# Whitby-Li/monoORBSLAM3

Measured on AMD Instinct MI355X. Metric: ORB extract+match frames/s @1242×375, 2000 feat; 1/2/4/8 GPU + %HBM roofline, higher is better.
Workload: dtype u8; 1 GPU; KITTI 1242x375, 2000 feat, 8-level pyramid scale 1.2, FAST 20/7; extract + 2000x2000 Hamming best-2 per frame; width=1242, height=375, n_features=2000, match=True, records=False, match_placement=after-fast, parallelism=512 resident frame(s) on one GPU, no collective

## Files before the change

### include/orbx.h

```cpp
#ifndef ORBX_H
#define ORBX_H

#include <stddef.h>
#include <stdint.h>

#ifdef __cplusplus
extern "C" {
#endif

#define ORBX_OK 0
#define ORBX_E_ARG (-1)
#define ORBX_E_NO_DEVICE (-2)
#define ORBX_E_CAPACITY (-3)
#define ORBX_E_UNSUPPORTED (-4)

#define ORBX_MAX_LEVELS 16

typedef struct orbx_kp {
    float x, y;
    float size;
    float angle;
    float response;
    int32_t octave;
    int32_t class_id;
// ... 38 lines not shown
int orbx_stream_wait_fast(orbx_t *h, void *stream);
int orbx_synchronize(orbx_t *h);
int orbx_host_register(void *ptr, size_t bytes);
int orbx_host_unregister(void *ptr);

int orbx_tap_level(orbx_t *h, int frame, int level, int blurred, uint8_t *out, size_t out_bytes);
int orbx_tap_candidates(orbx_t *h, int frame, int level, uint16_t *xs, uint16_t *ys, uint8_t *resp,
                        int cap, int *n_out);
int orbx_tap_level_counts(orbx_t *h, int frame, int32_t *counts);

int orbx_tap_sincos(orbx_t *h, const float *angles_deg, int n, float *cos_sin);

#define ORBX_VAR_FAST 0
#define ORBX_VAR_BLUR 1
#define ORBX_VAR_RESIZE_LDS 2
#define ORBX_VAR_RESIZE2 3
#define ORBX_VAR_SIDE_BLUR 4
#define ORBX_VAR_EARLY_FAST 5
#define ORBX_VAR_SPLIT_LEVEL0 6
#define ORBX_VAR_STREAMS 7
#define ORBX_VAR_ZERO_COPY 8
#define ORBX_VAR_DESC 9
#define ORBX_VAR_FAST_CELL_GROUP 10
#define ORBX_N_VARIANTS 11
int orbx_set_variant(orbx_t *h, int which, int value);
int orbx_get_variant(const orbx_t *h, int which, int *value);

#define ORBX_STAGE_RESIZE 0
#define ORBX_STAGE_FAST 1
#define ORBX_STAGE_BLUR 2
#define ORBX_STAGE_OCTREE 3
#define ORBX_STAGE_ORIENT 4
#define ORBX_STAGE_DESC 5
#define ORBX_N_STAGES 6
int orbx_set_stage_timing(orbx_t *h, int enable);
int orbx_stage_times_in_step_ms(orbx_t *h, float *ms );
int orbx_fast_times_in_step_ms(orbx_t *h, float *ms_sum, int *n_launches);
int orbx_stage_times_ms(orbx_t *h, float *ms );

const char *orbx_last_error(void);
const char *orbx_version(void);

#ifdef __cplusplus
}
#endif
#endif
```

### monoorbslam3_amd/csrc/orbx_api.hip

```cpp
#include <math.h>
#include <stdio.h>
#include <stdlib.h>
#include <string.h>

#include <algorithm>
#include <map>
#include <mutex>
#include <string>
#include <vector>

#include "orb_host.h"
#include "orb_math.h"
#include "orbx_internal.h"

static thread_local std::string g_err;
int orbx_set_error(int code, const std::string &msg) { g_err = msg; return code; }

hipError_t orbx_lds_opt_in(const void *kernel, size_t bytes)
{
    static std::mutex mu;
    static std::map<std::pair<const void *, int>, size_t> configured;
    int dev = 0;
    hipError_t e = hipGetDevice(&dev);
    if (e != hipSuccess) return e;
// ... 10 lines not shown
        sel, kp_ang, sel_count, sel_prefix, l0_stage;
};

struct orbx_ctx {
    orbx_cfg cfg;
    HandleStream hs;
    int n_cus = ORBX_N_CUS;
    float scale_factors[ORBX_MAX_LEVELS], inv_scale_factors[ORBX_MAX_LEVELS];
    float square_sigmas[ORBX_MAX_LEVELS], inv_square_sigmas[ORBX_MAX_LEVELS];
    float log_scale_factor;
    int quotas[ORBX_MAX_LEVELS];
    int u_max[ORBX_HALF_PATCH + 1];
    int taps[7];
    int cur_w, cur_h;
    OrbxLevels levels;
    size_t l0_stage_pitch;
    OrbxArenas arena;
    OrbxBuffers buf;
    DevBuf d_levels;
    DevBuf d_xtap[ORBX_MAX_LEVELS], d_ytap[ORBX_MAX_LEVELS];
    bool resize2_ok[ORBX_MAX_LEVELS];
    bool resize_lds_ok[ORBX_MAX_LEVELS];
    int resize_lds;
    int resize2;
    DevBuf d_umax, d_taps;
    hipEvent_t ev_after_fast; bool after_fast_valid;
    hipEvent_t ev_in[ORBX_N_STAGES][4]; int ev_in_n[ORBX_N_STAGES];
    DevBuf d_fast_cells; int n_fast_cells;
    DevBuf d_fast_strips; int n_fast_strips, n_fast_strips0;
    int fast_variant;
    int zero_copy;
    int fast_cell_group;
    int desc_variant;
    DevBuf d_blur_tiles; int n_blur_tiles;
    DevBuf d_blur_strips, d_band_h, d_band_v;
    BlurMfmaLevels blur_tab; int blur_strips_before[ORBX_MAX_LEVELS + 1]; int blur_mfma_levels;
    DevBuf d_bd_blocks, d_bd_band_h; int n_bd_blocks, bd_levels, bd_bk_stride;
    BdLevels bd_tab;
    DevBuf d_bd_bk_start, d_bd_items;
    int alloc_bd_batch, alloc_bd_kcap, alloc_bd_stride;
    int last_fused_levels;
    int blur_mfma;
    size_t l0_stage_fs;
    DevBuf d_slot_level;
    DevBuf d_out_block; PinBuf h_out_block; uint8_t *h_out_dev; size_t out_block_bytes, out_kp_off, out_desc_off;
    orbx_kp *d_out_kp; uint8_t *d_out_desc; int32_t *d_out_n;
// ... 67 lines not shown
}

static void linear_taps(int dn, int sn, bool clamp_ofs, std::vector<OrbxTap> &out)
{
    out.resize(dn);
    const double inv_scale = (double)dn / sn;
    const double scale = 1. / inv_scale;
    for (int d = 0; d < dn; ++d) {
        float f = (float)((d + 0.5) * scale - 0.5);
        int s = orb_floor_f(f);
        f -= (float)s;
        if (clamp_ofs) {
            if (s < 0) { f = 0; s = 0; }
            if (s >= sn - 1) { f = 0; s = sn - 1; }
        }
        auto sat = [](int v) { return (int16_t)std::min(std::max(v, -32768), 32767); };
        out[d].ofs = s;
        out[d].c0 = sat(orb_round_f((1.f - f) * 2048.f));
        out[d].c1 = sat(orb_round_f(f * 2048.f));
    }
}

static size_t align_up(size_t v, size_t a) { return (v + a - 1) / a * a; }
#ifndef ORBX_SIDE_FIRST_PIXELS
#define ORBX_SIDE_FIRST_PIXELS 1200000ull
#endif
#ifndef ORBX_FUSED_DESC_MIN_PIXELS
#define ORBX_FUSED_DESC_MIN_PIXELS 55000000ull
#endif

struct Geometry {
    OrbxLevels levels;
    size_t img_fs, cand_fs, node_fs, l0_fs;
    int l0_pitch;
    size_t sort_lds;
};

static int compute_geometry(const orbx_ctx *c, int w0, int h0, Geometry *g)
{
    memset(g, 0, sizeof *g);
    OrbxLevels &LV = g->levels;
    LV.n_levels = c->cfg.n_levels;
    LV.ini_th = c->cfg.ini_th_fast;
    LV.min_th = c->cfg.min_th_fast;
    size_t img = 0, cand = 0, node = 0;
    int kp = 0, max_quota = 1;
// ... 166 lines not shown
            std::vector<uint8_t> bh, bv;
            orbx_build_blur_mfma(c->levels, c->taps, bs, bh, bv, c->blur_tab, c->blur_strips_before);
            c->blur_mfma_levels = orbx_blur_mfma_levels(c->levels);
            ORB_TRY(upload(c->d_blur_strips, bs, 2));
            ORB_TRY(upload(c->d_band_h, bh, 16));
            ORB_TRY(upload(c->d_band_v, bv, 16));
            std::vector<uint16_t> bb;
            std::vector<uint8_t> bdh;
            orbx_build_blur_desc(c->levels, c->taps, c->blur_tab, bb, bdh, c->bd_tab, &c->bd_levels, &c->bd_bk_stride);
            c->n_bd_blocks = (int)(bb.size() / 2);
            ORB_TRY(upload(c->d_bd_blocks, bb, 2));
            ORB_TRY(upload(c->d_bd_band_h, bdh, 16));
        }
        std::vector<OrbxTap> taps, ytaps;
        for (int l = 1; l < c->levels.n_levels; ++l) {
            const OrbxLevel &d = c->levels.lv[l], &s = c->levels.lv[l - 1];
            linear_taps(d.w, s.w, true, taps);
            while (taps.size() % 4) taps.push_back(taps.back());
            ORB_TRY(upload(c->d_xtap[l], taps));
            linear_taps(d.h, s.h, false, ytaps);
            ORB_TRY(upload(c->d_ytap[l], ytaps));
            c->resize2_ok[l - 1] = l >= 2 && orbx_resize2_fits(taps.data(), ytaps.data(), s.w, s.h, d.w, d.h);
            c->resize_lds_ok[l] = orbx_resize_lds_fits(taps.data(), ytaps.data(), s.w, s.h, d.w, d.h);
        }
    }
    if (c->alloc_batch > c->alloc_bd_batch || c->levels.kcap_total > c->alloc_bd_kcap || c->bd_bk_stride > c->alloc_bd_stride) {
        ORB_TRY(hipDeviceSynchronize());
        c->alloc_bd_batch = std::max(c->alloc_batch, c->alloc_bd_batch);
        c->alloc_bd_kcap = std::max(c->levels.kcap_total, c->alloc_bd_kcap);
        c->alloc_bd_stride = std::max(c->bd_bk_stride, c->alloc_bd_stride);
        ORB_TRY(need_exact<int>(c->d_bd_bk_start, (size_t)c->alloc_bd_stride * c->alloc_bd_batch));
        ORB_TRY(need_exact<uint8_t>(c->d_bd_items, (size_t)32 * std::max(c->alloc_bd_kcap, 1) * c->alloc_bd_batch));
    }
    c->buf.img_frame_stride = c->alloc_img_fs;
    c->buf.cand_frame_stride = c->alloc_cand_fs;
    c->buf.node_frame_stride = c->alloc_node_fs;
    c->l0_stage_fs = c->alloc_l0_fs;
    return ORBX_OK;
}

static int create_common(const orbx_cfg *cfg, const int *quotas_override, orbx_t **out)
{
    if (!cfg || !out) return orbx_set_error(ORBX_E_ARG, "null argument");
    *out = nullptr;
    if (cfg->n_levels < 1 || cfg->n_levels > ORBX_MAX_LEVELS) return orbx_set_error(ORBX_E_ARG, "n_levels out of range");
    if (cfg->n_features < 1) return orbx_set_error(ORBX_E_ARG, "n_features must be >= 1");
// ... 18 lines not shown
        return cleanup(orbx_set_error(ORBX_E_NO_DEVICE, "hipStreamCreate failed"));
    for (int i = 0; i <= ORBX_N_STAGES; ++i)
        if (hipEventCreate(&c->ev[i]) != hipSuccess) return cleanup(orbx_set_error(ORBX_E_NO_DEVICE, "hipEventCreate failed"));
    for (int i = 0; i < 8; ++i)
        if (hipStreamCreateWithFlags(&c->sub[i], hipStreamNonBlocking) != hipSuccess ||
            hipEventCreateWithFlags(&c->ev_join[i], hipEventDisableTiming) != hipSuccess)
            return cleanup(orbx_set_error(ORBX_E_NO_DEVICE, "sub-stream creation failed"));
    if (hipEventCreateWithFlags(&c->ev_fork, hipEventDisableTiming) != hipSuccess)
        return cleanup(orbx_set_error(ORBX_E_NO_DEVICE, "hipEventCreate failed"));
    for (int i = 0; i < 9; ++i)
        if (hipStreamCreateWithFlags(&c->side[i], hipStreamNonBlocking) != hipSuccess ||
            hipEventCreateWithFlags(&c->ev_pyr[i], hipEventDisableTiming) != hipSuccess ||
            hipEventCreateWithFlags(&c->ev_blur[i], hipEventDisableTiming) != hipSuccess ||
            hipEventCreateWithFlags(&c->ev_start[i], hipEventDisableTiming) != hipSuccess ||
            hipEventCreateWithFlags(&c->ev_fast0[i], hipEventDisableTiming) != hipSuccess)
            return cleanup(orbx_set_error(ORBX_E_NO_DEVICE, "side-stream creation failed"));
    c->side_blur = 1;
    c->early_fast = -1;
    c->split_level0 = 1;
    c->fast_variant = 0;
    c->blur_mfma = 1;
    c->resize2 = 1;
    c->resize_lds = 1;
    c->n_sub = 1;
    c->zero_copy = 1;
    c->desc_variant = 0;
    c->fast_cell_group = 8;
    if (need_exact<OrbxLevels>(c->d_levels, 1) != hipSuccess || need_exact<int>(c->d_umax, 16) != hipSuccess ||
        need_exact<int>(c->d_taps, 8) != hipSuccess)
        return cleanup(orbx_set_error(ORBX_E_NO_DEVICE, "hipMalloc failed"));
    if (hipMemcpy(c->d_umax.p, c->u_max, sizeof(int) * 16, hipMemcpyHostToDevice) != hipSuccess ||
        hipMemcpy(c->d_taps.p, c->taps, sizeof(int) * 7, hipMemcpyHostToDevice) != hipSuccess)
        return cleanup(orbx_set_error(ORBX_E_NO_DEVICE, "hipMemcpy failed"));
    if (cfg->max_width > 0 && cfg->max_height > 0) {
        int rc = ensure_geometry(c, cfg->max_width, cfg->max_height, c->cfg.max_batch, 0);
        if (rc) return cleanup(rc);
    }
    *out = c;
    return ORBX_OK;
}

extern "C" int orbx_create(const orbx_cfg *cfg, orbx_t **out) { return create_common(cfg, nullptr, out); }


extern "C" int orbx_create_requota(const orbx_t *other, int n_features, orbx_t **out)
{
// ... 98 lines not shown
    const OrbxBuffers b = offset_buffers(c->buf, f0, LV.kcap_total);
    const OrbxLevels *d_levels = c->d_levels.as<OrbxLevels>();
    auto xtap = [&](int l) { return c->d_xtap[l].as<OrbxTap>(); };
    auto ytap = [&](int l) { return c->d_ytap[l].as<OrbxTap>(); };
    d_l0 += (size_t)f0 * l0_fs;
    d_kp += (size_t)f0 * cap; d_desc += (size_t)f0 * cap * 32; d_n += f0;
    if (t) ORB_TRY(hipEventRecord(c->ev[0], s));
    auto raw = [&](int l, const uint8_t **p, size_t *fs, int *pitch) {
        if (l == 0) { *p = d_l0; *fs = l0_fs; *pitch = l0_pitch; }
        else { *p = b.img_arena + LV.lv[l].raw_off; *fs = b.img_frame_stride; *pitch = LV.lv[l].pitch; }
    };
    const bool lds_resize = c->resize_lds == 2 || (c->resize_lds == 1 && (size_t)n_frames * (size_t)LV.lv[0].w * (size_t)LV.lv[0].h >= (size_t)100000000);
    auto launch_resize = [&](hipStream_t st, int l, int *zero_counts) -> int {
        const uint8_t *sp; size_t sfs; int spitch;
        raw(l - 1, &sp, &sfs, &spitch);
        if ((c->resize2 == 2 || (c->resize2 == 1 && n_frames < 24)) && l + 1 < L && c->resize2_ok[l] && LV.lv[l - 1].w >= 8) {
            orbx_launch_resize2(st, sp, sfs, spitch, LV.lv[l - 1].w, LV.lv[l - 1].h, b.img_arena + LV.lv[l].raw_off, b.img_frame_stride,
                                LV.lv[l].pitch, LV.lv[l].w, LV.lv[l].h, xtap(l), ytap(l), b.img_arena + LV.lv[l + 1].raw_off,
                                b.img_frame_stride, LV.lv[l + 1].pitch, LV.lv[l + 1].w, LV.lv[l + 1].h, xtap(l + 1),
                                ytap(l + 1), n_frames, zero_counts);
            return l + 1;
        }
        if (lds_resize && c->resize_lds_ok[l]) {
            orbx_launch_resize_lds(st, sp, sfs, spitch, LV.lv[l - 1].w, LV.lv[l - 1].h, l == 1 ? LV.lv[0].w : spitch,
                                   b.img_arena + LV.lv[l].raw_off, b.img_frame_stride, LV.lv[l].pitch, LV.lv[l].w, LV.lv[l].h, xtap(l),
                                   ytap(l), n_frames, zero_counts);
            return l;
        }
        orbx_launch_resize(st, sp, sfs, spitch, LV.lv[l - 1].w, LV.lv[l - 1].h, b.img_arena + LV.lv[l].raw_off, b.img_frame_stride,
                           LV.lv[l].pitch, LV.lv[l].w, LV.lv[l].h, xtap(l), ytap(l), n_frames, zero_counts);
        return l;
    };
    const bool side_ok = !t && c->side_blur && slot >= 0;
    const bool strips = c->fast_variant == 2 || (c->fast_variant == 0 && n_frames >= 24);
    const uint16_t *d_units = (strips ? c->d_fast_strips : c->d_fast_cells).as<uint16_t>();
    const int n_units = strips ? c->n_fast_strips : c->n_fast_cells;
    const int n_cells0 = strips ? c->n_fast_strips0 : LV.lv[0].n_cols * LV.lv[0].n_rows;
    auto launch_fast = [&](hipStream_t st, const uint16_t *units, int n) {
        InStep ft(c, ORBX_STAGE_FAST, st);
        if (strips) orbx_launch_fast_strips(st, d_l0, l0_fs, l0_pitch, d_levels, LV, b, units, n, n_frames);
        else orbx_launch_fast(st, d_l0, l0_fs, l0_pitch, d_levels, LV, b, units, n, n_frames, c->fast_cell_group);
    };
    const bool big_call = (size_t)n_frames * (size_t)LV.lv[0].w * (size_t)LV.lv[0].h >= (size_t)ORBX_FUSED_DESC_MIN_PIXELS;
    const int fl = (c->desc_variant == 2 || (c->desc_variant == 0 && big_call)) ? c->bd_levels : 0;
    c->last_fused_levels = fl;
    auto launch_blur = [&](hipStream_t st, int lb, int le) {
        lb = std::max(lb, fl);
        if (le <= lb) return;
        InStep bt(c, ORBX_STAGE_BLUR, st);
// ... 398 lines not shown
{
    if (!c || !ms) return orbx_set_error(ORBX_E_ARG, "null argument");
    if (!c->ev_valid) return orbx_set_error(ORBX_E_ARG, "no timed extract call yet");
    ORB_TRY(hipSetDevice(c->hs.device));
    ORB_TRY(hipEventSynchronize(c->ev[ORBX_N_STAGES]));
    for (int i = 0; i < ORBX_N_STAGES; ++i) ORB_TRY(hipEventElapsedTime(&ms[i], c->ev[i], c->ev[i + 1]));
    return ORBX_OK;
}

static int *variant_field(orbx_ctx *c, int which, int *lo, int *hi)
{
    switch (which) {
    case ORBX_VAR_FAST: *lo = 0; *hi = 2; return &c->fast_variant;
    case ORBX_VAR_BLUR: *lo = 0; *hi = 2; return &c->blur_mfma;
    case ORBX_VAR_RESIZE_LDS: *lo = 0; *hi = 2; return &c->resize_lds;
    case ORBX_VAR_RESIZE2: *lo = 0; *hi = 2; return &c->resize2;
    case ORBX_VAR_SIDE_BLUR: *lo = 0; *hi = 3; return &c->side_blur;
    case ORBX_VAR_EARLY_FAST: *lo = -1; *hi = 2; return &c->early_fast;
    case ORBX_VAR_SPLIT_LEVEL0: *lo = 0; *hi = ORBX_MAX_LEVELS; return &c->split_level0;
    case ORBX_VAR_STREAMS: *lo = 1; *hi = 8; return &c->n_sub;
    case ORBX_VAR_ZERO_COPY: *lo = 0; *hi = 1; return &c->zero_copy;
    case ORBX_VAR_DESC: *lo = 0; *hi = 2; return &c->desc_variant;
    case ORBX_VAR_FAST_CELL_GROUP: *lo = 1; *hi = 16; return &c->fast_cell_group;
    default: return nullptr;
    }
}

extern "C" int orbx_set_variant(orbx_t *c, int which, int value)
{
    if (!c) return orbx_set_error(ORBX_E_ARG, "null handle");
    int lo, hi;
    int *f = variant_field(c, which, &lo, &hi);
    if (!f) return orbx_set_error(ORBX_E_ARG, "unknown variant switch");
    if (value < lo || value > hi) return orbx_set_error(ORBX_E_ARG, "variant value out of range");
    if (which == ORBX_VAR_FAST_CELL_GROUP && value != 1 && value != 4 && value != 8 && value != 16)
        return orbx_set_error(ORBX_E_ARG, "FAST cell group must be 1, 4, 8 or 16");
    if (which == ORBX_VAR_SPLIT_LEVEL0 && value > c->cfg.n_levels - 1)
        return orbx_set_error(ORBX_E_ARG, "split level must be below the handle's n_levels");
    *f = value;
    return ORBX_OK;
}

extern "C" int orbx_get_variant(const orbx_t *c, int which, int *value)
{
    if (!c || !value) return orbx_set_error(ORBX_E_ARG, "null argument");
    int lo, hi;
// ... 15 lines not shown
    ORB_TRY(hipHostUnregister(ptr));
    return ORBX_OK;
}

extern "C" int orbx_dev_octree_plan(const orbx_cfg *cfg, int requota, int w0, int h0, int n_frames, int level_begin, int level_end,
                                    int64_t *out)
{
    if (!cfg || !out || cfg->n_levels < 1 || cfg->n_levels > ORBX_MAX_LEVELS || cfg->n_features < 1 || !(cfg->scale_factor > 1.0f))
        return orbx_set_error(ORBX_E_ARG, "bad argument");
    if (level_begin < 0 || level_end > cfg->n_levels || level_end <= level_begin || n_frames < 1) return orbx_set_error(ORBX_E_ARG, "bad level range");
    orbx_ctx *c = new orbx_ctx();
    c->cfg = *cfg;
    compute_tables(c);
    if (requota > 0) compute_quotas(c, requota);
    Geometry g;
    int rc = compute_geometry(c, w0, h0, &g);
    delete c;
    if (rc) return rc;
    const OrbxOctPlan p = orbx_octree_plan(g.levels, n_frames, level_begin, level_end);
    out[0] = p.kind; out[1] = (int64_t)p.lds_bytes; out[2] = (int64_t)p.huge_bytes; out[3] = p.huge_end;
    return ORBX_OK;
}

extern "C" int orbx_dev_xcd_map(int per_frame, int n_frames, int block_id, int *frame, int *item)
{
    if (per_frame < 1 || n_frames < 1 || !frame || !item) return orbx_set_error(ORBX_E_ARG, "bad argument");
    const int rc = orbx_xcd_map_query(per_frame, n_frames, block_id, frame, item);
    return rc < 0 ? orbx_set_error(ORBX_E_ARG, "block outside the grid") : rc;
}

extern "C" const char *orbx_last_error(void) { return g_err.c_str(); }
extern "C" const char *orbx_version(void) { return "orbx 0.1 (gfx950)"; }

#ifdef OCT_PROF
unsigned long long *orbx_dev_fast_prof_symbol();
extern "C" int orbx_dev_fast_prof(orbx_t *c, unsigned long long *out16, int reset)
{
    if (!c || !out16) return orbx_set_error(ORBX_E_ARG, "null argument");
    ORB_TRY(hipSetDevice(c->hs.device));
    ORB_TRY(hipDeviceSynchronize());
    unsigned long long *sym = orbx_dev_fast_prof_symbol();
    if (!sym) return orbx_set_error(ORBX_E_ARG, "no counter symbol");
    ORB_TRY(hipMemcpy(out16, sym, sizeof(unsigned long long) * 16, hipMemcpyDeviceToHost));
    if (reset) ORB_TRY(hipMemset(sym, 0, sizeof(unsigned long long) * 16));
    return ORBX_OK;
}
// ... 22 lines not shown
```

### monoorbslam3_amd/csrc/orbx_internal.h

```cpp
#pragma once
#include <hip/hip_runtime.h>
#include <stddef.h>
#include <stdint.h>

#include <vector>

#include "../../include/orbx.h"
#include "orb_host.h"

#define ORBX_EDGE 19
#define ORBX_CELL 30
#define ORBX_HALF_PATCH 15
#ifndef ORBX_OCT_THREADS
#define ORBX_OCT_THREADS 512
#endif
#ifndef ORBX_OCT_THREADS_BATCH
#define ORBX_OCT_THREADS_BATCH 256
#endif

struct OrbxLevel {
    int w, h;
    int pitch;
    int n_cols, n_rows;
    int region_w, region_h;
// ... 24 lines not shown

struct OrbxBuffers {
    uint8_t *img_arena;        size_t img_frame_stride;
    unsigned long long *cand;  size_t cand_frame_stride;
    int *cand_count;
    uint32_t *pnode;
    uint32_t *pcode;
    size_t node_frame_stride;
    short4 *bnd0, *bnd1;
    int *cnt0, *cnt1;
    int *rank, *node_of_rank, *newpos;
    int *childcnt, *childpos;
    unsigned long long *best;
    uint2 *sel;
    int *sel_count;
    int *sel_prefix;
    const int *slot_level;
    float4 *kp_ang;
};

void orbx_launch_resize(hipStream_t s, const uint8_t *src, size_t src_fs, int src_pitch, int sw, int sh,
                        uint8_t *dst, size_t dst_fs, int dst_pitch, int dw, int dh,
                        const OrbxTap *xtap, const OrbxTap *ytap, int n_frames, int *zero_counts = nullptr);
bool orbx_resize_lds_fits(const OrbxTap *xtap, const OrbxTap *ytap, int sw, int sh, int dw, int dh);
void orbx_launch_resize_lds(hipStream_t s, const uint8_t *src, size_t src_fs, int src_pitch, int sw, int sh, int last_row_bytes,
                            uint8_t *dst, size_t dst_fs, int dst_pitch, int dw, int dh, const OrbxTap *xtap, const OrbxTap *ytap,
                            int n_frames, int *zero_counts);
bool orbx_resize2_fits(const OrbxTap *xtap2, const OrbxTap *ytap2, int w1, int h1, int w2, int h2);
void orbx_launch_resize2(hipStream_t s, const uint8_t *src, size_t src_fs, int src_pitch, int sw, int sh, uint8_t *d1, size_t d1_fs,
                         int d1_pitch, int w1, int h1, const OrbxTap *xtap1, const OrbxTap *ytap1, uint8_t *d2, size_t d2_fs,
                         int d2_pitch, int w2, int h2, const OrbxTap *xtap2, const OrbxTap *ytap2, int n_frames, int *zero_counts);
void orbx_launch_fast(hipStream_t s, const uint8_t *l0, size_t l0_fs, int l0_pitch, const OrbxLevels *d_levels,
                      const OrbxLevels &levels, const OrbxBuffers &b, const void *d_cells, int n_cells, int n_frames,
                      int cells_per_group);
int orbx_build_fast_cells(const OrbxLevels &levels, uint16_t *out);
int orbx_build_fast_strips(const OrbxLevels &levels, int level_begin, int level_end, uint16_t *out);
void orbx_launch_fast_strips(hipStream_t s, const uint8_t *l0, size_t l0_fs, int l0_pitch, const OrbxLevels *d_levels,
                             const OrbxLevels &levels, const OrbxBuffers &b, const void *d_strips, int n_strips, int n_frames);
void orbx_launch_blur(hipStream_t s, const uint8_t *l0, size_t l0_fs, int l0_pitch, const OrbxLevels *d_levels,
                      const OrbxLevels &levels, const OrbxBuffers &b, const void *d_tiles, int n_tiles, const int *taps7,
                      int n_frames, int level_begin, int level_end);
int orbx_build_blur_tiles(const OrbxLevels &levels, uint16_t *out);
struct BlurMfmaLevels {
    int w[ORBX_MAX_LEVELS], h[ORBX_MAX_LEVELS], dst_pitch[ORBX_MAX_LEVELS], n_ty[ORBX_MAX_LEVELS];
    unsigned long long dst_off[ORBX_MAX_LEVELS];
    int bh_off[ORBX_MAX_LEVELS], bv_off[ORBX_MAX_LEVELS];
};
int orbx_blur_mfma_levels(const OrbxLevels &levels);
void orbx_build_blur_mfma(const OrbxLevels &levels, const int taps[7], std::vector<uint16_t> &strips, std::vector<uint8_t> &band_h,
                          std::vector<uint8_t> &band_v, BlurMfmaLevels &out, int strips_before[ORBX_MAX_LEVELS + 1]);
// ... 31 lines not shown
```

### monoorbslam3_amd/csrc/orbx_kernels.hip

```cpp
#include <string.h>

#include <vector>

#include "orbx_internal.h"
#include <atomic>
#include "orb_math.h"
#include "orb_pattern.h"

typedef unsigned long long u64;

__host__ __device__ __forceinline__ bool orbx_xcd_map(int id, int per_frame, int n_frames, int *frame, int *item)
{
    if (n_frames < 8) {
        const int f = id / per_frame;
        *item = id - f * per_frame;
        *frame = f;
        return f < n_frames;
    }
    const int xcd = id & 7, j = id >> 3;
    const int g = j / per_frame;
    *item = j - g * per_frame;
    *frame = g * 8 + xcd;
    return *frame < n_frames;
}
// ... 111 lines not shown
__device__ __forceinline__ uint32_t resize_quad(uint32_t w0l, uint32_t w0h, uint32_t w1l, uint32_t w1h, const uint32_t sel[4],
                                                const uint32_t cc[4], int b0, int b1)
{
    typedef unsigned short u16x2 __attribute__((ext_vector_type(2)));
    uint32_t packed = 0;
#pragma unroll
    for (int i = 0; i < 4; ++i) {
        const u16x2 cv = __builtin_bit_cast(u16x2, cc[i]);
        const int r0 = (int)__builtin_amdgcn_udot2(__builtin_bit_cast(u16x2, __builtin_amdgcn_perm(w0h, w0l, sel[i])), cv, 0u, false);
        const int r1 = (int)__builtin_amdgcn_udot2(__builtin_bit_cast(u16x2, __builtin_amdgcn_perm(w1h, w1l, sel[i])), cv, 0u, false);
        const int v = (((int)__umul24((uint32_t)b0, (uint32_t)(r0 >> 4)) >> 16) + ((int)__umul24((uint32_t)b1, (uint32_t)(r1 >> 4)) >> 16) + 2) >> 2;
        packed |= (uint32_t)v << (8 * i);
    }
    return packed;
}

#define RL_NC 22
#define RL_LP (RL_NC * 16 + 16)
#ifndef RL_WAVES
#define RL_WAVES 4
#endif
#define RL_NR (RL_WAVES * 10 + 2)
#define RL_ROUNDS ((RL_NR + 2 * RL_WAVES - 1) / (2 * RL_WAVES))
__global__ __launch_bounds__(64 * RL_WAVES) void k_resize_lds(const uint8_t *__restrict__ src, size_t src_fs, int src_pitch, int sw,
                                                    int sh, int last_row_bytes, uint8_t *__restrict__ dst, size_t dst_fs,
                                                    int dst_pitch, int dw, int dh, const OrbxTap *__restrict__ xtap,
                                                    const OrbxTap *__restrict__ ytap, int gx, int gy, int n_frames,
                                                    int *__restrict__ zero_counts)
{
    __shared__ __align__(16) uint8_t tile[RL_NR * RL_LP];
    int frame, blk;
    if (!xcd_remap(gx * gy, n_frames, &frame, &blk)) return;
    const int tid = threadIdx.y * 64 + threadIdx.x;
    if (zero_counts && blk == 0 && tid < ORBX_MAX_LEVELS) zero_counts[frame * ORBX_MAX_LEVELS + tid] = 0;
    const int by = blk / gx, bx = blk - by * gx;
    const int X0 = bx * 256, Y0 = by * RL_WAVES * RS_ROWS, Xl = min(X0 + 255, dw - 1), Yl = min(Y0 + RL_WAVES * RS_ROWS - 1, dh - 1);
    const int colbase = xtap[X0].ofs & ~15;
    const int ncol = ((min(xtap[Xl].ofs + 1, sw - 1) - colbase) >> 4) + 1;
    const int r_lo = min(max(ytap[Y0].ofs, 0), sh - 1);
    const int nrow = min(max(ytap[Yl].ofs + 1, 0), sh - 1) - r_lo + 1;
    const uint8_t *S = src + (size_t)frame * src_fs;
    uint8_t *D = dst + (size_t)frame * dst_fs;
    {
        struct __attribute__((packed, aligned(1))) U128 { uint32_t w[4]; };
        const int ch = tid & 31, rs = tid >> 5;
        U128 v[RL_ROUNDS];
        bool slow[RL_ROUNDS];
#pragma unroll
        for (int k = 0; k < RL_ROUNDS; ++k) {
            const int row = rs + 2 * RL_WAVES * k, y = r_lo + row, c = colbase + 16 * ch;
            const bool on = ch < ncol && row < nrow;
            slow[k] = on && y == sh - 1 && c + 16 > last_row_bytes;
            v[k].w[0] = v[k].w[1] = v[k].w[2] = v[k].w[3] = 0;
            if (on && !slow[k]) v[k] = *reinterpret_cast<const U128 *>(S + (size_t)y * src_pitch + c);
            if (slow[k])
                for (int q = 0; q < 16; ++q)
                    if (c + q < last_row_bytes) v[k].w[q >> 2] |= (uint32_t)S[(size_t)y * src_pitch + c + q] << (8 * (q & 3));
// ... 44 lines not shown
            rowA = r0;
        }
        if (r1 != rowB) {
            if (r1 == rowA) {
#pragma unroll
                for (int i = 0; i < 4; ++i) gB[i] = gA[i];
            } else {
                hrow(r1, gB);
            }
            rowB = r1;
        }
        uint32_t sm[4];
#pragma unroll
        for (int i = 0; i < 4; ++i) {
            const uint32_t p0 = __umul24((uint32_t)ty.c0, gA[i]) + 0x20000u, p1 = __umul24((uint32_t)ty.c1, gB[i]);
            asm("v_add_u32_sdwa %0, %1, %2 dst_sel:DWORD dst_unused:UNUSED_PAD src0_sel:WORD_1 src1_sel:WORD_1" : "=v"(sm[i]) : "v"(p0), "v"(p1));
        }
        const rl_u16x2 lo = __builtin_bit_cast(rl_u16x2, __builtin_amdgcn_perm(sm[1], sm[0], 0x05040100u)) >> (unsigned short)2;
        const rl_u16x2 hi = __builtin_bit_cast(rl_u16x2, __builtin_amdgcn_perm(sm[3], sm[2], 0x05040100u)) >> (unsigned short)2;
        const uint32_t q = __builtin_amdgcn_perm(__builtin_bit_cast(uint32_t, hi), __builtin_bit_cast(uint32_t, lo), 0x06040200u);
        *reinterpret_cast<uint32_t *>(D + (size_t)(dy0 + r) * dst_pitch + dx0) = q;
    }
}
bool orbx_resize_lds_fits(const OrbxTap *xtap, const OrbxTap *ytap, int sw, int sh, int dw, int dh)
{
    for (int X0 = 0; X0 < dw; X0 += 256) {
        const int Xl = std::min(X0 + 255, dw - 1), colbase = xtap[X0].ofs & ~15;
        if (xtap[X0].ofs < 0 || ((std::min(xtap[Xl].ofs + 1, sw - 1) - colbase) >> 4) + 1 > RL_NC) return false;
    }
    for (int Y0 = 0; Y0 < dh; Y0 += RL_WAVES * RS_ROWS) {
        const int Yl = std::min(Y0 + RL_WAVES * RS_ROWS - 1, dh - 1);
        const int r_lo = std::min(std::max(ytap[Y0].ofs, 0), sh - 1);
        if (std::min(std::max(ytap[Yl].ofs + 1, 0), sh - 1) - r_lo + 1 > RL_NR) return false;
    }
    return sw >= 16;
}
void orbx_launch_resize_lds(hipStream_t s, const uint8_t *src, size_t src_fs, int src_pitch, int sw, int sh, int last_row_bytes,
                            uint8_t *dst, size_t dst_fs, int dst_pitch, int dw, int dh, const OrbxTap *xtap, const OrbxTap *ytap,
                            int n_frames, int *zero_counts)
{
    const int gx = (dw + 255) / 256, gy = (dh + RL_WAVES * RS_ROWS - 1) / (RL_WAVES * RS_ROWS);
    hipLaunchKernelGGL(k_resize_lds, dim3(orbx_xcd_grid(gx * gy, n_frames)), dim3(64, RL_WAVES), dev_pad(k_resize_lds, 0, 0), s, src, src_fs, src_pitch, sw, sh,
                       last_row_bytes, dst, dst_fs, dst_pitch, dw, dh, xtap, ytap, gx, gy, n_frames, zero_counts);
}

#define R2_TW 64
#define R2_TH 16
#define R2_RW 104
#define R2_RH 24
struct Resize2Args {
    const uint8_t *src; size_t src_fs; int src_pitch, sw, sh;
    uint8_t *d1; size_t d1_fs; int d1_pitch, w1, h1; const OrbxTap *xtap1, *ytap1;
    uint8_t *d2; size_t d2_fs; int d2_pitch, w2, h2; const OrbxTap *xtap2, *ytap2;
    int gx, gy, n_frames; int *zero_counts;
};
__global__ __launch_bounds__(256) void k_resize2(Resize2Args a)
{
    __shared__ __align__(16) uint8_t patch[R2_RH * R2_RW];
    int frame, blk;
    if (!xcd_remap(a.gx * a.gy, a.n_frames, &frame, &blk)) return;
    const int tid = threadIdx.x;
    if (a.zero_counts && blk == 0 && tid < ORBX_MAX_LEVELS) a.zero_counts[frame * ORBX_MAX_LEVELS + tid] = 0;
    const int by = blk / a.gx, bx = blk - by * a.gx;
    const int X0 = bx * R2_TW, Y0 = by * R2_TH, X1 = min(X0 + R2_TW, a.w2), Y1 = min(Y0 + R2_TH, a.h2);
    const int cb = a.xtap2[X0].ofs & ~3;
    const int cn = bx + 1 < a.gx ? (a.xtap2[X0 + R2_TW].ofs & ~3) : ((a.w1 + 3) & ~3);
// ... 2029 lines not shown
```

### monoorbslam3_amd/extractor.py

```python
import ctypes as C

import numpy as np

from . import _lib

KP_DTYPE = np.dtype([("x", "<f4"), ("y", "<f4"), ("size", "<f4"), ("angle", "<f4"), ("response", "<f4"),
                     ("octave", "<i4"), ("class_id", "<i4")])
STAGES = ("resize", "fast", "blur", "octree", "orient", "desc")
VARIANTS = {
    "fast": (0, {"auto": 0, "cells": 1, "strips": 2}),
    "blur": (1, {"valu": 0, "auto": 1, "mfma": 2}),
    "resize_lds": (2, {"never": 0, "auto": 1, "always": 2}),
    "resize2": (3, {"never": 0, "auto": 1, "always": 2}),
    "side_blur": (4, {}),
    "early_fast": (5, {"auto": -1}),
    "split_level0": (6, {}),
    "streams": (7, {}),
    "zero_copy": (8, {}),
    "desc": (9, {"auto": 0, "separate": 1, "fused": 2}),
    "fast_cell_group": (10, {}),
}


def _vp(a):
    return a.ctypes.data_as(C.c_void_p)


class ORBExtractor:

    def __init__(self, nFeatures=1000, scaleFactor=1.2, nLevels=8, iniThFast=20, minThFast=10, *, max_width=0,
                 max_height=0, max_batch=1, blur_variant=0, device=-1, variants=None, _requota_of=None):
        self._L = _lib.lib()
        self._h = C.c_void_p()
        if _requota_of is not None:
            _lib.check(self._L.orbx_create_requota(_requota_of._h, nFeatures, C.byref(self._h)))
        else:
            cfg = _lib.OrbxCfg(nFeatures, scaleFactor, nLevels, iniThFast, minThFast, max_width, max_height,
                               max_batch, blur_variant, device)
            _lib.check(self._L.orbx_create(C.byref(cfg), C.byref(self._h)))
        n = C.c_int()
        self._sf = np.zeros(_lib.MAX_LEVELS, np.float32)
        self._isf = np.zeros(_lib.MAX_LEVELS, np.float32)
        self._ss = np.zeros(_lib.MAX_LEVELS, np.float32)
# ... 173 lines not shown
```

Baseline: 249,500 frames/s.

## Pack resize remainder columns into dedicated tall-narrow LDS tiles

Adds a remainder path to the LDS resize kernel. When a level's width is not a multiple of 256, the leftover columns are handled by extra blocks that cover 64-row bands split into up to 4 column slabs, instead of full 256-wide tiles that are mostly empty. Outputs are staged through LDS and written back as coalesced 32-bit stores. This is meant to cut wasted work and loads on partial tiles, at the cost of more blocks per frame and extra synchronisation inside the remainder blocks.

Result: no change. 251,700 frames/s (median of 6 runs) (+0.9%).

```diff
diff --git a/include/orbx.h b/include/orbx.h
--- a/include/orbx.h
+++ b/include/orbx.h
@@ -84,7 +84,8 @@
 #define ORBX_VAR_ZERO_COPY 8
 #define ORBX_VAR_DESC 9
 #define ORBX_VAR_FAST_CELL_GROUP 10
-#define ORBX_N_VARIANTS 11
+#define ORBX_VAR_RESIZE_REM 11
+#define ORBX_N_VARIANTS 12
 int orbx_set_variant(orbx_t *h, int which, int value);
 int orbx_get_variant(const orbx_t *h, int which, int *value);
 
diff --git a/monoorbslam3_amd/csrc/orbx_api.hip b/monoorbslam3_amd/csrc/orbx_api.hip
--- a/monoorbslam3_amd/csrc/orbx_api.hip
+++ b/monoorbslam3_amd/csrc/orbx_api.hip
@@ -56,6 +56,8 @@
     bool resize2_ok[ORBX_MAX_LEVELS];
     bool resize_lds_ok[ORBX_MAX_LEVELS];
     int resize_lds;
+    int rem_ns[ORBX_MAX_LEVELS], rem_gs[ORBX_MAX_LEVELS];
+    int resize_rem;
     int resize2;
     DevBuf d_umax, d_taps;
     hipEvent_t ev_after_fast; bool after_fast_valid;
@@ -169,6 +171,12 @@
 }
 
 static size_t align_up(size_t v, size_t a) { return (v + a - 1) / a * a; }
+static const int ORBX_RESIZE_REM_MAX_GROUPS = 28;
+static bool resize_rem_packed(int mode, int dw, int rem_ns)
+{
+    const int ng = (dw % 256 + 3) / 4;
+    return rem_ns > 0 && (mode == 2 || (mode == 1 && ng <= ORBX_RESIZE_REM_MAX_GROUPS));
+}
 #ifndef ORBX_SIDE_FIRST_PIXELS
 #define ORBX_SIDE_FIRST_PIXELS 1200000ull
 #endif
@@ -381,6 +389,8 @@
             ORB_TRY(upload(c->d_ytap[l], ytaps));
             c->resize2_ok[l - 1] = l >= 2 && orbx_resize2_fits(taps.data(), ytaps.data(), s.w, s.h, d.w, d.h);
             c->resize_lds_ok[l] = orbx_resize_lds_fits(taps.data(), ytaps.data(), s.w, s.h, d.w, d.h);
+            if (!c->resize_lds_ok[l] || !orbx_resize_rem_plan(taps.data(), ytaps.data(), s.w, s.h, d.w, d.h, &c->rem_ns[l], &c->rem_gs[l]))
+                c->rem_ns[l] = c->rem_gs[l] = 0;
         }
     }
     if (c->alloc_batch > c->alloc_bd_batch || c->levels.kcap_total > c->alloc_bd_kcap || c->bd_bk_stride > c->alloc_bd_stride) {
@@ -445,6 +455,7 @@
     c->blur_mfma = 1;
     c->resize2 = 1;
     c->resize_lds = 1;
+    c->resize_rem = 1;
     c->n_sub = 1;
     c->zero_copy = 1;
     c->desc_variant = 0;
@@ -589,9 +600,10 @@
             return l + 1;
         }
         if (lds_resize && c->resize_lds_ok[l]) {
+            const bool packed = resize_rem_packed(c->resize_rem, LV.lv[l].w, c->rem_ns[l]);
             orbx_launch_resize_lds(st, sp, sfs, spitch, LV.lv[l - 1].w, LV.lv[l - 1].h, l == 1 ? LV.lv[0].w : spitch,
                                    b.img_arena + LV.lv[l].raw_off, b.img_frame_stride, LV.lv[l].pitch, LV.lv[l].w, LV.lv[l].h, xtap(l),
-                                   ytap(l), n_frames, zero_counts);
+                                   ytap(l), n_frames, zero_counts, packed ? c->rem_ns[l] : 0, packed ? c->rem_gs[l] : 0);
             return l;
         }
         orbx_launch_resize(st, sp, sfs, spitch, LV.lv[l - 1].w, LV.lv[l - 1].h, b.img_arena + LV.lv[l].raw_off, b.img_frame_stride,
@@ -1036,6 +1048,7 @@
     case ORBX_VAR_ZERO_COPY: *lo = 0; *hi = 1; return &c->zero_copy;
     case ORBX_VAR_DESC: *lo = 0; *hi = 2; return &c->desc_variant;
     case ORBX_VAR_FAST_CELL_GROUP: *lo = 1; *hi = 16; return &c->fast_cell_group;
+    case ORBX_VAR_RESIZE_REM: *lo = 0; *hi = 2; return &c->resize_rem;
     default: return nullptr;
     }
 }
@@ -1097,6 +1110,32 @@
     return ORBX_OK;
 }
 
+extern "C" int orbx_dev_resize_rem_plan(const orbx_cfg *cfg, int w0, int h0, int mode, int32_t *out)
+{
+    if (!cfg || !out || cfg->n_levels < 1 || cfg->n_levels > ORBX_MAX_LEVELS || cfg->n_features < 1 || !(cfg->scale_factor > 1.0f) || mode < 0 || mode > 2)
+        return orbx_set_error(ORBX_E_ARG, "bad argument");
+    orbx_ctx *c = new orbx_ctx();
+    c->cfg = *cfg;
+    compute_tables(c);
+    Geometry g;
+    int rc = compute_geometry(c, w0, h0, &g);
+    delete c;
+    if (rc) return rc;
+    std::vector<OrbxTap> taps, ytaps;
+    out[0] = out[1] = 0;
+    for (int l = 1; l < g.levels.n_levels; ++l) {
+        const OrbxLevel &d = g.levels.lv[l], &s = g.levels.lv[l - 1];
+        linear_taps(d.w, s.w, true, taps);
+        while (taps.size() % 4) taps.push_back(taps.back());
+        linear_taps(d.h, s.h, false, ytaps);
+        int ns = 0, gs = 0;
+        const bool ok = orbx_resize_lds_fits(taps.data(), ytaps.data(), s.w, s.h, d.w, d.h) &&
+                        orbx_resize_rem_plan(taps.data(), ytaps.data(), s.w, s.h, d.w, d.h, &ns, &gs) && resize_rem_packed(mode, d.w, ns);
+        out[2 * l] = ok ? ns : 0; out[2 * l + 1] = ok ? gs : 0;
+    }
+    return ORBX_OK;
+}
+
 extern "C" int orbx_dev_xcd_map(int per_frame, int n_frames, int block_id, int *frame, int *item)
 {
     if (per_frame < 1 || n_frames < 1 || !frame || !item) return orbx_set_error(ORBX_E_ARG, "bad argument");
diff --git a/monoorbslam3_amd/csrc/orbx_internal.h b/monoorbslam3_amd/csrc/orbx_internal.h
--- a/monoorbslam3_amd/csrc/orbx_internal.h
+++ b/monoorbslam3_amd/csrc/orbx_internal.h
@@ -70,10 +70,11 @@
 void orbx_launch_resize(hipStream_t s, const uint8_t *src, size_t src_fs, int src_pitch, int sw, int sh,
                         uint8_t *dst, size_t dst_fs, int dst_pitch, int dw, int dh,
                         const OrbxTap *xtap, const OrbxTap *ytap, int n_frames, int *zero_counts = nullptr);
-bool orbx_resize_lds_fits(const OrbxTap *xtap, const OrbxTap *ytap, int sw, int sh, int dw, int dh);
+bool orbx_resize_lds_fits(const OrbxTap *xtap, const OrbxTap *ytap, int sw, int sh, int dw, int dh, int rem_ns = 0, int rem_gs = 0);
+bool orbx_resize_rem_plan(const OrbxTap *xtap, const OrbxTap *ytap, int sw, int sh, int dw, int dh, int *rem_ns, int *rem_gs);
 void orbx_launch_resize_lds(hipStream_t s, const uint8_t *src, size_t src_fs, int src_pitch, int sw, int sh, int last_row_bytes,
                             uint8_t *dst, size_t dst_fs, int dst_pitch, int dw, int dh, const OrbxTap *xtap, const OrbxTap *ytap,
-                            int n_frames, int *zero_counts);
+                            int n_frames, int *zero_counts, int rem_ns = 0, int rem_gs = 0);
 bool orbx_resize2_fits(const OrbxTap *xtap2, const OrbxTap *ytap2, int w1, int h1, int w2, int h2);
 void orbx_launch_resize2(hipStream_t s, const uint8_t *src, size_t src_fs, int src_pitch, int sw, int sh, uint8_t *d1, size_t d1_fs,
                          int d1_pitch, int w1, int h1, const OrbxTap *xtap1, const OrbxTap *ytap1, uint8_t *d2, size_t d2_fs,
diff --git a/monoorbslam3_amd/csrc/orbx_kernels.hip b/monoorbslam3_amd/csrc/orbx_kernels.hip
--- a/monoorbslam3_amd/csrc/orbx_kernels.hip
+++ b/monoorbslam3_amd/csrc/orbx_kernels.hip
@@ -157,17 +157,121 @@
 #endif
 #define RL_NR (RL_WAVES * 10 + 2)
 #define RL_ROUNDS ((RL_NR + 2 * RL_WAVES - 1) / (2 * RL_WAVES))
+#define RP_ROWS 64
+#define RP_NC 11
+#define RP_LP (RP_NC * 16 + 4)
+#define RP_NR ((RL_NR * RL_LP) / RP_LP)
+#define RP_ROUNDS ((RP_NR + 4 * RL_WAVES - 1) / (4 * RL_WAVES))
+#define RP_MAX_SLABS 4
+#define RP_GW 9
+static_assert(RP_NR * RP_LP + 8 <= RL_NR * RL_LP && RP_LP % 8 == 4 && RP_ROWS * (RL_WAVES * RP_GW + 1) * 4 <= RL_NR * RL_LP, "k_resize_lds: packed remainder layout");
+__device__ __forceinline__ void resize_lds_rem(uint8_t *tile, const uint8_t *__restrict__ S, int src_pitch, int sw, int sh, int last_row_bytes,
+                                               uint8_t *__restrict__ D, int dst_pitch, int dw, int dh, const OrbxTap *__restrict__ xtap,
+                                               const OrbxTap *__restrict__ ytap, int Xr, int rb, int rem_ns, int rem_gs)
+{
+    typedef unsigned short rl_u16x2 __attribute__((ext_vector_type(2)));
+    const int tid = threadIdx.y * 64 + threadIdx.x;
+    const int band = rb / rem_ns, slab = rb - band * rem_ns;
+    const int ng = (dw - Xr + 3) >> 2, g0 = slab * rem_gs, g1 = min(g0 + rem_gs, ng);
+    const int Xs = Xr + 4 * g0, Xl = min(Xr + 4 * g1 - 1, dw - 1);
+    const int Y0 = band * RP_ROWS, Yl = min(Y0 + RP_ROWS - 1, dh - 1);
+    const int colbase = xtap[Xs].ofs & ~15;
+    const int ncol = ((min(xtap[Xl].ofs + 1, sw - 1) - colbase) >> 4) + 1;
+    const int r_lo = min(max(ytap[Y0].ofs, 0), sh - 1);
+    const int nrow = min(max(ytap[Yl].ofs + 1, 0), sh - 1) - r_lo + 1;
+    {
+        struct __attribute__((packed, aligned(1))) U128 { uint32_t w[4]; };
+        const int ch = tid & 15, rs = tid >> 4;
+        U128 v[RP_ROUNDS];
+        bool slow[RP_ROUNDS];
+#pragma unroll
+        for (int k = 0; k < RP_ROUNDS; ++k) {
+            const int row = rs + 4 * RL_WAVES * k, y = r_lo + row, c = colbase + 16 * ch;
+            const bool on = ch < ncol && row < nrow;
+            slow[k] = on && y == sh - 1 && c + 16 > last_row_bytes;
+            v[k].w[0] = v[k].w[1] = v[k].w[2] = v[k].w[3] = 0;
+            if (on && !slow[k]) v[k] = *reinterpret_cast<const U128 *>(S + (size_t)y * src_pitch + c);
+            if (slow[k])
+                for (int q = 0; q < 16; ++q)
+                    if (c + q < last_row_bytes) v[k].w[q >> 2] |= (uint32_t)S[(size_t)y * src_pitch + c + q] << (8 * (q & 3));
+        }
+#pragma unroll
+        for (int k = 0; k < RP_ROUNDS; ++k) {
+            const int row = rs + 4 * RL_WAVES * k;
+            if (ch < ncol && row < nrow) {
+                uint32_t *t = reinterpret_cast<uint32_t *>(&tile[row * RP_LP + 16 * ch]);
+                t[0] = v[k].w[0]; t[1] = v[k].w[1]; t[2] = v[k].w[2]; t[3] = v[k].w[3];
+            }
+        }
+    }
+    __syncthreads();
+    const int y = min(Y0 + (int)threadIdx.x, dh - 1);
+    const OrbxTap ty = ytap[y];
+    const uint8_t *p0 = tile + (min(max(ty.ofs, 0), sh - 1) - r_lo) * RP_LP, *p1 = tile + (min(max(ty.ofs + 1, 0), sh - 1) - r_lo) * RP_LP;
+    const uint32_t b0 = ty.c0, b1 = ty.c1;
+    auto quad = [&](int g) -> uint32_t {
+        const int dx0 = Xr + 4 * g;
+        const uint4 t01 = reinterpret_cast<const uint4 *>(xtap + dx0)[0], t23 = reinterpret_cast<const uint4 *>(xtap + dx0)[1];
+        const int ofs[4] = {(int)t01.x, (int)t01.z, (int)t23.x, (int)t23.z};
+        const uint32_t cc[4] = {t01.y, t01.w, t23.y, t23.w};
+        const int a = ofs[0] - colbase;
+        const uint32_t sh8 = (uint32_t)(a & 3) * 8u;
+        uint32_t sel[4];
+#pragma unroll
+        for (int i = 0; i < 4; ++i) sel[i] = (uint32_t)(ofs[i] - ofs[0]) * 0x00010001u + 0x0c010c00u;
+        const uint32_t *q0 = reinterpret_cast<const uint32_t *>(p0 + (a & ~3)), *q1 = reinterpret_cast<const uint32_t *>(p1 + (a & ~3));
+        const uint32_t a0 = q0[0], a1 = q0[1], a2 = q0[2], c0 = q1[0], c1 = q1[1], c2 = q1[2];
+        const uint32_t wl0 = __builtin_amdgcn_alignbit(a1, a0, sh8), wh0 = __builtin_amdgcn_alignbit(a2, a1, sh8);
+        const uint32_t wl1 = __builtin_amdgcn_alignbit(c1, c0, sh8), wh1 = __builtin_amdgcn_alignbit(c2, c1, sh8);
+        uint32_t sm[4];
+#pragma unroll
+        for (int i = 0; i < 4; ++i) {
+            const uint32_t h0 = __builtin_amdgcn_udot2(__builtin_bit_cast(rl_u16x2, __builtin_amdgcn_perm(wh0, wl0, sel[i])), __builtin_bit_cast(rl_u16x2, cc[i]), 0u, false) >> 4;
+            const uint32_t h1 = __builtin_amdgcn_udot2(__builtin_bit_cast(rl_u16x2, __builtin_amdgcn_perm(wh1, wl1, sel[i])), __builtin_bit_cast(rl_u16x2, cc[i]), 0u, false) >> 4;
+            const uint32_t m0 = __umul24(b0, h0) + 0x20000u, m1 = __umul24(b1, h1);
+            asm("v_add_u32_sdwa %0, %1, %2 dst_sel:DWORD dst_unused:UNUSED_PAD src0_sel:WORD_1 src1_sel:WORD_1" : "=v"(sm[i]) : "v"(m0), "v"(m1));
+        }
+        const rl_u16x2 lo = __builtin_bit_cast(rl_u16x2, __builtin_amdgcn_perm(sm[1], sm[0], 0x05040100u)) >> (unsigned short)2;
+        const rl_u16x2 hi = __builtin_bit_cast(rl_u16x2, __builtin_amdgcn_perm(sm[3], sm[2], 0x05040100u)) >> (unsigned short)2;
+        return __builtin_amdgcn_perm(__builtin_bit_cast(uint32_t, hi), __builtin_bit_cast(uint32_t, lo), 0x06040200u);
+    };
+    const int wave = __builtin_amdgcn_readfirstlane((int)threadIdx.y);
+    uint32_t q[RP_GW];
+#pragma unroll
+    for (int k = 0; k < RP_GW; ++k) {
+        q[k] = 0;
+        if (g0 + wave + RL_WAVES * k < g1) q[k] = quad(g0 + wave + RL_WAVES * k);
+    }
+    __syncthreads();
+    const int nsl = g1 - g0, op = nsl | 1;
+    uint32_t *out = reinterpret_cast<uint32_t *>(tile);
+#pragma unroll
+    for (int k = 0; k < RP_GW; ++k)
+        if (g0 + wave + RL_WAVES * k < g1) out[(int)threadIdx.x * op + wave + RL_WAVES * k] = q[k];
+    __syncthreads();
+    const uint32_t inv = ((1u << 20) + (uint32_t)nsl - 1u) / (uint32_t)nsl;
+    for (int i = tid; i < RP_ROWS * nsl; i += 64 * RL_WAVES) {
+        const int row = (int)(((uint32_t)i * inv) >> 20), col = i - row * nsl;
+        if (Y0 + row < dh) *reinterpret_cast<uint32_t *>(D + (size_t)(Y0 + row) * dst_pitch + Xs + 4 * col) = out[row * op + col];
+    }
+}
+
 __global__ __launch_bounds__(64 * RL_WAVES) void k_resize_lds(const uint8_t *__restrict__ src, size_t src_fs, int src_pitch, int sw,
                                                     int sh, int last_row_bytes, uint8_t *__restrict__ dst, size_t dst_fs,
                                                     int dst_pitch, int dw, int dh, const OrbxTap *__restrict__ xtap,
                                                     const OrbxTap *__restrict__ ytap, int gx, int gy, int n_frames,
-                                                    int *__restrict__ zero_counts)
+                                                    int *__restrict__ zero_counts, int rem_ns, int rem_gs)
 {
     __shared__ __align__(16) uint8_t tile[RL_NR * RL_LP];
     int frame, blk;
-    if (!xcd_remap(gx * gy, n_frames, &frame, &blk)) return;
+    if (!xcd_remap(gx * gy + rem_ns * ((dh + RP_ROWS - 1) / RP_ROWS), n_frames, &frame, &blk)) return;
     const int tid = threadIdx.y * 64 + threadIdx.x;
     if (zero_counts && blk == 0 && tid < ORBX_MAX_LEVELS) zero_counts[frame * ORBX_MAX_LEVELS + tid] = 0;
+    if (blk >= gx * gy) {
+        resize_lds_rem(tile, src + (size_t)frame * src_fs, src_pitch, sw, sh, last_row_bytes, dst + (size_t)frame * dst_fs, dst_pitch, dw, dh,
+                       xtap, ytap, 256 * gx, blk - gx * gy, rem_ns, rem_gs);
+        return;
+    }
     const int by = blk / gx, bx = blk - by * gx;
     const int X0 = bx * 256, Y0 = by * RL_WAVES * RS_ROWS, Xl = min(X0 + 255, dw - 1), Yl = min(Y0 + RL_WAVES * RS_ROWS - 1, dh - 1);
     const int colbase = xtap[X0].ofs & ~15;
@@ -258,26 +362,52 @@
         *reinterpret_cast<uint32_t *>(D + (size_t)(dy0 + r) * dst_pitch + dx0) = q;
     }
 }
-bool orbx_resize_lds_fits(const OrbxTap *xtap, const OrbxTap *ytap, int sw, int sh, int dw, int dh)
-{
-    for (int X0 = 0; X0 < dw; X0 += 256) {
+bool orbx_resize_lds_fits(const OrbxTap *xtap, const OrbxTap *ytap, int sw, int sh, int dw, int dh, int rem_ns, int rem_gs)
+{
+    const int Xr = rem_ns > 0 ? dw / 256 * 256 : dw;
+    for (int X0 = 0; X0 < Xr; X0 += 256) {
         const int Xl = std::min(X0 + 255, dw - 1), colbase = xtap[X0].ofs & ~15;
         if (xtap[X0].ofs < 0 || ((std::min(xtap[Xl].ofs + 1, sw - 1) - colbase) >> 4) + 1 > RL_NC) return false;
     }
-    for (int Y0 = 0; Y0 < dh; Y0 += RL_WAVES * RS_ROWS) {
+    for (int Y0 = 0; Y0 < dh && Xr > 0; Y0 += RL_WAVES * RS_ROWS) {
         const int Yl = std::min(Y0 + RL_WAVES * RS_ROWS - 1, dh - 1);
         const int r_lo = std::min(std::max(ytap[Y0].ofs, 0), sh - 1);
         if (std::min(std::max(ytap[Yl].ofs + 1, 0), sh - 1) - r_lo + 1 > RL_NR) return false;
     }
+    if (rem_ns > 0) {
+        const int ng = (dw - Xr + 3) / 4;
+        if (ng < 1 || rem_gs < 1 || rem_gs > RL_WAVES * RP_GW || rem_ns > RP_MAX_SLABS || rem_ns * rem_gs < ng || (rem_ns - 1) * rem_gs >= ng) return false;
+        for (int g0 = 0; g0 < ng; g0 += rem_gs) {
+            const int Xs = Xr + 4 * g0, Xl = std::min(Xr + 4 * std::min(g0 + rem_gs, ng) - 1, dw - 1), colbase = xtap[Xs].ofs & ~15;
+            if (xtap[Xs].ofs < 0 || ((std::min(xtap[Xl].ofs + 1, sw - 1) - colbase) >> 4) + 1 > RP_NC) return false;
+        }
+        for (int Y0 = 0; Y0 < dh; Y0 += RP_ROWS) {
+            const int Yl = std::min(Y0 + RP_ROWS - 1, dh - 1);
+            const int r_lo = std::min(std::max(ytap[Y0].ofs, 0), sh - 1);
+            if (std::min(std::max(ytap[Yl].ofs + 1, 0), sh - 1) - r_lo + 1 > RP_NR) return false;
+        }
+    }
     return sw >= 16;
+}
+bool orbx_resize_rem_plan(const OrbxTap *xtap, const OrbxTap *ytap, int sw, int sh, int dw, int dh, int *rem_ns, int *rem_gs)
+{
+    const int ng = (dw % 256 + 3) / 4;
+    for (int ns = 1; ns <= RP_MAX_SLABS && ng > 0; ++ns) {
+        const int gs = (ng + ns - 1) / ns;
+        if ((ns - 1) * gs >= ng) continue;
+        if (orbx_resize_lds_fits(xtap, ytap, sw, sh, dw, dh, ns, gs)) { *rem_ns = ns; *rem_gs = gs; return true; }
+    }
+    *rem_ns = *rem_gs = 0;
+    return false;
 }
 void orbx_launch_resize_lds(hipStream_t s, const uint8_t *src, size_t src_fs, int src_pitch, int sw, int sh, int last_row_bytes,
                             uint8_t *dst, size_t dst_fs, int dst_pitch, int dw, int dh, const OrbxTap *xtap, const OrbxTap *ytap,
-                            int n_frames, int *zero_counts)
-{
-    const int gx = (dw + 255) / 256, gy = (dh + RL_WAVES * RS_ROWS - 1) / (RL_WAVES * RS_ROWS);
-    hipLaunchKernelGGL(k_resize_lds, dim3(orbx_xcd_grid(gx * gy, n_frames)), dim3(64, RL_WAVES), dev_pad(k_resize_lds, 0, 0), s, src, src_fs, src_pitch, sw, sh,
-                       last_row_bytes, dst, dst_fs, dst_pitch, dw, dh, xtap, ytap, gx, gy, n_frames, zero_counts);
+                            int n_frames, int *zero_counts, int rem_ns, int rem_gs)
+{
+    const int gx = rem_ns > 0 ? dw / 256 : (dw + 255) / 256, gy = (dh + RL_WAVES * RS_ROWS - 1) / (RL_WAVES * RS_ROWS);
+    const int per_frame = gx * gy + rem_ns * ((dh + RP_ROWS - 1) / RP_ROWS);
+    hipLaunchKernelGGL(k_resize_lds, dim3(orbx_xcd_grid(per_frame, n_frames)), dim3(64, RL_WAVES), dev_pad(k_resize_lds, 0, 0), s, src, src_fs, src_pitch, sw, sh,
+                       last_row_bytes, dst, dst_fs, dst_pitch, dw, dh, xtap, ytap, gx, gy, n_frames, zero_counts, rem_ns, rem_gs);
 }
 
 #define R2_TW 64
diff --git a/monoorbslam3_amd/extractor.py b/monoorbslam3_amd/extractor.py
--- a/monoorbslam3_amd/extractor.py
+++ b/monoorbslam3_amd/extractor.py
@@ -19,6 +19,7 @@
     "zero_copy": (8, {}),
     "desc": (9, {"auto": 0, "separate": 1, "fused": 2}),
     "fast_cell_group": (10, {}),
+    "resize_rem": (11, {"never": 0, "auto": 1, "always": 2}),
 }
 
 
```
